# nicholasburden/pymarl

Hardware: NVIDIA B200
Metric: qmix_learner_episodes_per_sec (higher is better)
Workload: dtype bf16 (fp32 accumulate)

## Files before the change

pymarl_b200/csrc/api.cu:

```cuda
#include <cstdlib>
#include <stdarg.h>
#include <string.h>
#include <stdlib.h>
#include <atomic>
#include <mutex>
#include <vector>
#include <cuda_bf16.h>
#include "common.cuh"
#include "gru_tc.cuh"
#include "mixer_tc.cuh"

namespace pmb {

int gru_fwd_dispatch(const pmb_dims* d, const AgentParams& p, int64_t R, int nt, const float* x, const float* h0,
                     float* h_stash, float* gates, float* q, float* h_last, cudaStream_t s);
int gru_bwd_dispatch(const pmb_dims* d, const pmb_batch* b, const AgentParams& p, const float* x,
                     const float* h_stash, float* gates, const float* d_chosen, float* dpre1, cudaStream_t s,
                     const float* dq_full = nullptr);
int64_t scatter_scratch_bytes(const pmb_dims* d);
int scatter_grads_dispatch(const pmb_dims* d, const pmb_batch* b, const float* h_stash, const float* dpre1,
                           const float* d_chosen, AgentGrads gr, void* scratch, int64_t scratch_bytes, cudaStream_t s,
                           int ti_tiles = 0);
int launch_target_select(const pmb_dims* d, const pmb_batch* b, const float* q_on, const float* q_tg, float* chosen,
                         float* tmax, int32_t* cur_max, cudaStream_t s);
// ... 222 lines not shown
        T * R * A,
        T * R * A,
        M * N,
        M * N,
        qmix ? (tc_mix ? tc_raw_img_bytes(d) / 4 : M * C) : 0,
        (d->precision == PMB_PREC_BF16 && d->H == 64) ? T * n_tiles * ((d->O + 63) / 64) * ti : 0,
        iql ? 0 : M,
        iql ? 0 : M,
        M * W,
        iql ? 0 : M * N,
        tc_mix ? tc_state_img_bytes(d) / 4 : 0,
        (d->precision == PMB_PREC_BF16 && d->H == 64) ? (T + 1) * n_tiles * ti : 0,
        (d->precision == PMB_PREC_BF16 && d->H == 64) ? T * n_tiles * 256 : 0,
        0
    };
    WsPlan p;
    int64_t off = 0;
    for (int i = 0; i < 17; ++i) {
        p.off[i] = off;
        off += align_up(sizes[i] * 4, 256);
    }
    int64_t sc = agent_bwd_scratch(d);
    int64_t mb = mixer_bwd_scratch_bytes(d);
    if (mb > sc) sc = mb;
    if (d->precision == PMB_PREC_BF16) {
        int64_t f = tc_fc1_scratch_bytes(d);
        if (f > sc) sc = f;
        int64_t g = 131072 + tc_gru_bwd2_partial_bytes((int)ceil_div((int64_t)d->B * d->N, 128));
        if (g > sc) sc = g;
        int64_t a2 = tc_atb_ti_scratch_bytes(d->T, (int)ceil_div((int64_t)d->B * d->N, 128), d->O);
        if (a2 > sc) sc = a2;
        if (tc_agent_dw_scratch_bytes() > sc) sc = tc_agent_dw_scratch_bytes();
        if (tc_mix) {
            int64_t m2 = tc_mixer_scratch_bytes(d); if (m2 > sc) sc = m2;
            int64_t m3 = tc_mixer_bwd_img_scratch_bytes(d); if (m3 > sc) sc = m3;
        }
    }
    if (sc < 65536) sc = 65536;
    p.off[17] = off;
    p.scratch_bytes = align_up(sc, 256);
    p.mixdw_bytes = (tc_mix && d->H == 64) ? tc_mixer_dw_scratch_bytes(d) : 0;
    p.sched_bytes = skip_padding(d) ? skip_schedule_bytes(d->B, d->T, (int)n_tiles) : 0;
    p.total = off + p.scratch_bytes + p.mixdw_bytes + p.sched_bytes;
    return p;
}

void fill_views(const pmb_dims* d, void* ws, const WsPlan& p, pmb_ws_views* v) {
    char* base = static_cast<char*>(ws);
    auto f = [&](int i) { return reinterpret_cast<float*>(base + p.off[i]); };
    const bool iql = d->mixer == PMB_MIXER_NONE;
    v->x_on = f(0); v->x_tg = f(1); v->h_stash = f(2); v->gates = f(3); v->q_on = f(4); v->q_tg = f(5);
    v->chosen = f(6); v->tmax = f(7); v->raw_on = f(8); v->raw_tg = f(8);
    v->q_tot = iql ? v->chosen : f(10);
    v->t_tot = iql ? v->tmax : f(11);
    v->g = f(12);
    v->d_chosen = iql ? v->g : f(13);
    v->scratch = f(17);
    v->relu_mask = f(16);
    v->state_img = f(14);
    v->h_tg = f(15);
    v->scratch_bytes = p.scratch_bytes;
    v->obs_img = f(9);
    v->ep_order = nullptr;
    v->tile_steps = nullptr;
    if (p.sched_bytes) {
        SkipSchedule S = skip_schedule_views(base + p.total - p.sched_bytes, d->B, d->T, (int)ceil_div((int64_t)d->B * d->N, 128));
        v->ep_order = S.ep_order;
// ... 429 lines not shown
        }
        if ((rc = tc_gru_fwd2(img(0), img(24576), on.b_ih, on.b_hh, x_on_ti, h_ti, g_ti, R, d->T, n_tiles, s, tpc, tile_steps)))
            return rc;
        if (fork_tg) {
            PMB_CUDA(cudaStreamWaitEvent(s, side->join, 0));
        } else {
            PHASE(s, "gru_unroll_fwd_target_tc");
            if ((rc = tc_gru_fwd2(img(57344), img(57344 + 24576), tg.b_ih, tg.b_hh, x_tg_ti, hg_ti, nullptr, R, d->T, n_tiles,
                                  s, 2, tile_steps))) return rc;
        }
        PHASE(s, "q_select_tc");
        if ((rc = tc_q_select(d, b, img(49152), img(57344 + 49152), on.fc2_b, tg.fc2_b, h_ti, hg_ti, n_tiles, v.chosen,
                              v.tmax, (hp->keep_q & 1) ? v.q_on : nullptr, (hp->keep_q & 1) ? v.q_tg : nullptr, s, live_items,
                              n_live, tile_steps))) return rc;
    } else {
        PHASE(s, "fc1_fwd_online");
        if ((rc = fc1_fwd(d, b, 0, d->T, on, v.x_on, s))) return rc;
        PHASE(s, "fc1_fwd_target");
        if ((rc = fc1_fwd(d, b, 0, d->T, tg, v.x_tg, s))) return rc;
    }
    if (!tc_agent) {
        PHASE(s, "gru_unroll_fwd_online");
        if ((rc = gru_fwd_dispatch(d, on, R, d->T, v.x_on, nullptr, v.h_stash, v.gates, v.q_on, nullptr, s))) return rc;
        PHASE(s, "gru_unroll_fwd_target");
        if ((rc = gru_fwd_dispatch(d, tg, R, d->T, v.x_tg, nullptr, nullptr, nullptr, v.q_tg, nullptr, s))) return rc;
    }
    if (!tc_agent) {
        PHASE(s, "target_select");
        if ((rc = launch_target_select(d, b, v.q_on, v.q_tg, v.chosen, v.tmax, nullptr, s))) return rc;
    }
    uint8_t* state_img = reinterpret_cast<uint8_t*>(v.state_img);
    uint8_t* raw_img = reinterpret_cast<uint8_t*>(v.raw_on);
    if (tc_mixer) {
        PHASE(s, "state_to_images");
        if ((rc = tc_state_to_images(d, b, state_img, s))) return rc;
        PHASE(s, "mixer_fwd_target_tc");
        if ((rc = tc_mixer_fwd_img(d, mixer_params(d, flat_target + L.n_agent), state_img, v.tmax, 1, nullptr, v.t_tot,
                                   v.scratch, v.scratch_bytes, s))) return rc;
        PHASE(s, "mixer_fwd_online_tc");
        if ((rc = tc_mixer_fwd_img(d, mixer_params(d, flat_p + L.n_agent), state_img, v.chosen, 0, raw_img, v.q_tot,
                                   v.scratch, v.scratch_bytes, s))) return rc;
    } else if (d->mixer != PMB_MIXER_NONE) {
        PHASE(s, "mixer_fwd_target");
        if ((rc = launch_mixer_fwd(d, b, flat_target + L.n_agent, v.tmax, 1, v.raw_tg, v.t_tot, s))) return rc;
        PHASE(s, "mixer_fwd_online");
        if ((rc = launch_mixer_fwd(d, b, flat_p + L.n_agent, v.chosen, 0, v.raw_on, v.q_tot, s))) return rc;
    }
    PHASE(s, "td_loss");
    if ((rc = launch_td_loss(d, b, v.q_tot, v.t_tot, hp->gamma, v.g, stats, s, reinterpret_cast<double*>(v.scratch),
                             v.scratch_bytes))) return rc;
    if (hp->keep_q & 2) {
        PHASE(s, "end");
        return PMB_OK;
    }
    PHASE(s, "mixer_bwd");
    SideStream* side_dw = nullptr;
    if (tc_mixer) {
        static const int dw_fork_mode = []() { const char* e = getenv("PMB_DW_FORK"); return e ? atoi(e) : -1; }();
        const int free_sms = sm_count() - n_tiles;
        const bool fork_dw = tc_agent && plan.mixdw_bytes > 0 && dw_fork_mode != 0 && free_sms >= tc_mixer_dw_ctas(d);
        if (!fork_dw) {
            if ((rc = tc_mixer_bwd_img(d, mixer_params(d, flat_p + L.n_agent), state_img, raw_img, v.chosen, v.g, v.d_chosen,
                                       flat_g + L.offset[PMB_P_HW1_W], flat_g + L.offset[PMB_P_HW1_B],
                                       flat_g + L.offset[PMB_P_V2_W], flat_g + L.offset[PMB_P_V2_B], v.scratch,
                                       v.scratch_bytes, s))) return rc;
        } else {
            if ((rc = tc_mixer_bwd_img_dq(d, mixer_params(d, flat_p + L.n_agent), raw_img, v.chosen, v.g, v.d_chosen,
                                          flat_g + L.offset[PMB_P_V2_W], flat_g + L.offset[PMB_P_V2_B], v.scratch,
                                          v.scratch_bytes, s))) return rc;
            if ((rc = side_stream(&side_dw))) return rc;
            PMB_CUDA(cudaEventRecord(side_dw->fork2, s));
            PMB_CUDA(cudaStreamWaitEvent(side_dw->stream, side_dw->fork2, 0));
            if ((rc = tc_mixer_dw(d, state_img, raw_img, flat_g + L.offset[PMB_P_HW1_W], flat_g + L.offset[PMB_P_HW1_B],
                                  reinterpret_cast<char*>(v.scratch) + plan.scratch_bytes, plan.mixdw_bytes, free_sms,
// ... 253 lines not shown
```

pymarl_b200/csrc/mixer_tc.cuh:

```cuda
#pragma once
#include <cuda_bf16.h>
#include "common.cuh"

namespace pmb {

int64_t tc_packed_elems(int Ncols, int K);
int tc_pack_w(const float* const* ptrs, const int* rows, const int* lds, int nseg, int K, __nv_bfloat16* out,
              cudaStream_t s, int n_chunks_min = 0);

inline int tc_state_chunks(const pmb_dims* d) { return (d->S + 1 + 63) / 64; }
inline int tc_mix_cblks(const pmb_dims* d) { return (d->N + 3 + 1) / 2; }
inline int64_t tc_mix_row_tiles(const pmb_dims* d) { return ((int64_t)d->B * d->T + 127) / 128; }
inline int64_t tc_state_img_bytes(const pmb_dims* d) { return tc_mix_row_tiles(d) * tc_state_chunks(d) * 16384; }
inline int64_t tc_raw_img_bytes(const pmb_dims* d) { return tc_mix_row_tiles(d) * tc_mix_cblks(d) * 16384; }

int64_t tc_mixer_scratch_bytes(const pmb_dims* d);
int tc_state_to_images(const pmb_dims* d, const pmb_batch* b, uint8_t* img, cudaStream_t s);
int tc_mixer_fwd_img(const pmb_dims* d, const MixerParams& mp, const uint8_t* state_img, const float* agent_qs, int t_off,
                     uint8_t* raw_img, float* q_tot, void* scratch, int64_t scratch_bytes, cudaStream_t s);

int64_t tc_mixer_bwd_img_scratch_bytes(const pmb_dims* d);
int tc_mixer_bwd_img_dq(const pmb_dims* d, const MixerParams& mp, uint8_t* raw_img, const float* agent_qs, const float* g,
                        float* d_agent_qs, float* gv2_w, float* gv2_b, void* scratch, int64_t scratch_bytes, cudaStream_t s);
int tc_mixer_dw_ctas(const pmb_dims* d);
int64_t tc_mixer_dw_scratch_bytes(const pmb_dims* d);
int tc_mixer_dw(const pmb_dims* d, const uint8_t* state_img, const uint8_t* raw_img, float* gw_cat, float* gb_cat,
                void* scratch, int64_t scratch_bytes, int ctas_avail, cudaStream_t s);
int tc_mixer_bwd_img(const pmb_dims* d, const MixerParams& mp, const uint8_t* state_img, uint8_t* raw_img,
                     const float* agent_qs, const float* g, float* d_agent_qs, float* gw_cat, float* gb_cat, float* gv2_w,
                     float* gv2_b, void* scratch, int64_t scratch_bytes, cudaStream_t s);

}
```

pymarl_b200/csrc/tc_common.cuh:

```cuda
#pragma once
#include <cuda_bf16.h>
#include <stdint.h>

namespace pmb {
namespace tc {

__device__ __forceinline__ uint32_t smem_u32(const void* p) { return (uint32_t)__cvta_generic_to_shared(p); }

__device__ __forceinline__ void mbar_init(uint64_t* bar, uint32_t count) {
    asm volatile("mbarrier.init.shared::cta.b64 [%0], %1;" ::"r"(smem_u32(bar)), "r"(count) : "memory");
}
__device__ __forceinline__ void fence_barrier_init() {
    asm volatile("fence.mbarrier_init.release.cluster;" ::: "memory");
}
__device__ __forceinline__ void mbar_arrive(uint64_t* bar) {
    asm volatile("mbarrier.arrive.shared::cta.b64 _, [%0];" ::"r"(smem_u32(bar)) : "memory");
}
__device__ __forceinline__ void mbar_arrive_expect_tx(uint64_t* bar, uint32_t bytes) {
    asm volatile("mbarrier.arrive.expect_tx.shared::cta.b64 _, [%0], %1;" ::"r"(smem_u32(bar)), "r"(bytes) : "memory");
}
__device__ __forceinline__ bool mbar_try_wait(uint64_t* bar, uint32_t parity) {
    uint32_t ok;
    asm volatile(
        "{\n\t.reg .pred p;\n\t"
// ... 4 lines not shown
        : "memory");
    return ok != 0;
}
__device__ __forceinline__ void mbar_wait(uint64_t* bar, uint32_t parity) {
    while (!mbar_try_wait(bar, parity)) {
    }
}

typedef unsigned long long f32x2;
__device__ __forceinline__ f32x2 f2_make(float lo, float hi) {
    f32x2 r;
    asm("mov.b64 %0, {%1, %2};" : "=l"(r) : "f"(lo), "f"(hi));
    return r;
}
__device__ __forceinline__ void f2_split(f32x2 v, float& lo, float& hi) { asm("mov.b64 {%0, %1}, %2;" : "=f"(lo), "=f"(hi) : "l"(v)); }
__device__ __forceinline__ f32x2 f2_from_bf16x2(uint32_t w) { return f2_make(__uint_as_float(w << 16), __uint_as_float(w & 0xffff0000u)); }
__device__ __forceinline__ f32x2 f2_fma(f32x2 a, f32x2 b, f32x2 c) {
    f32x2 d;
    asm("fma.rn.f32x2 %0, %1, %2, %3;" : "=l"(d) : "l"(a), "l"(b), "l"(c));
    return d;
}
__device__ __forceinline__ f32x2 f2_mul(f32x2 a, f32x2 b) {
    f32x2 d;
    asm("mul.rn.f32x2 %0, %1, %2;" : "=l"(d) : "l"(a), "l"(b));
    return d;
}
__device__ __forceinline__ f32x2 f2_add(f32x2 a, f32x2 b) {
    f32x2 d;
    asm("add.rn.f32x2 %0, %1, %2;" : "=l"(d) : "l"(a), "l"(b));
    return d;
}

__device__ __forceinline__ void fence_proxy_async_smem() { asm volatile("fence.proxy.async.shared::cta;" ::: "memory"); }

__device__ __forceinline__ void bulk_copy_g2s(void* dst_smem, const void* src_gmem, uint32_t bytes, uint64_t* bar) {
    asm volatile("cp.async.bulk.shared::cluster.global.mbarrier::complete_tx::bytes [%0], [%1], %2, [%3];" ::"r"(
                     smem_u32(dst_smem)),
                 "l"(src_gmem), "r"(bytes), "r"(smem_u32(bar))
                 : "memory");
}

__device__ __forceinline__ void bulk_copy_s2g(void* dst_gmem, const void* src_smem, uint32_t bytes) {
    asm volatile("cp.async.bulk.global.shared::cta.bulk_group [%0], [%1], %2;" ::"l"(dst_gmem), "r"(smem_u32(src_smem)),
                 "r"(bytes)
                 : "memory");
}
__device__ __forceinline__ void bulk_commit_group() { asm volatile("cp.async.bulk.commit_group;" ::: "memory"); }
template <int N>
__device__ __forceinline__ void bulk_wait_group_read() { asm volatile("cp.async.bulk.wait_group.read %0;" ::"n"(N) : "memory"); }
template <int N>
__device__ __forceinline__ void bulk_wait_group() { asm volatile("cp.async.bulk.wait_group %0;" ::"n"(N) : "memory"); }

__device__ __forceinline__ void tmem_alloc(uint32_t* slot_smem, uint32_t ncols) {
    asm volatile("tcgen05.alloc.cta_group::1.sync.aligned.shared::cta.b32 [%0], %1;" ::"r"(smem_u32(slot_smem)), "r"(ncols)
                 : "memory");
    asm volatile("tcgen05.relinquish_alloc_permit.cta_group::1.sync.aligned;" ::: "memory");
}
__device__ __forceinline__ void tmem_dealloc(uint32_t taddr, uint32_t ncols) {
    asm volatile("tcgen05.dealloc.cta_group::1.sync.aligned.b32 %0, %1;" ::"r"(taddr), "r"(ncols) : "memory");
}
__device__ __forceinline__ void pdl_launch_dependents() { asm volatile("griddepcontrol.launch_dependents;" ::: "memory"); }
__device__ __forceinline__ void pdl_wait() { asm volatile("griddepcontrol.wait;" ::: "memory"); }

__device__ __forceinline__ void tc_fence_before() { asm volatile("tcgen05.fence::before_thread_sync;" ::: "memory"); }
__device__ __forceinline__ void tc_fence_after() { asm volatile("tcgen05.fence::after_thread_sync;" ::: "memory"); }
__device__ __forceinline__ void tmem_wait_ld() { asm volatile("tcgen05.wait::ld.sync.aligned;" ::: "memory"); }
// ... 75 lines not shown
```

pymarl_b200/csrc/tc_gemm.cu:

```cuda
#include <cstdlib>
#include <algorithm>
#include "common.cuh"
#include "tc_common.cuh"
#include "mixer_tc.cuh"

namespace pmb {
namespace tc {

constexpr int BM = 128;
constexpr int BK = 64;
constexpr int BN_MAX = 256;
constexpr int STAGES = 4;
constexpr int A_STAGE_BYTES = BM * 128;
constexpr int W_STAGE_BYTES = BN_MAX * 128;
constexpr int N_EPI_WARPS = 4, MMA_WARP = 4, WLOAD_WARP = 5, FIRST_PROD_WARP = 6, N_PROD_WARPS = 8;
constexpr int THREADS = 32 * (FIRST_PROD_WARP + N_PROD_WARPS);
constexpr int SMEM_BYTES = 1024  + STAGES * (A_STAGE_BYTES + W_STAGE_BYTES) + 256;

struct GemmParams {
    const float* A;
    RowMap amap;
    int64_t M;
    int K;
    int n_chunks;
    const __nv_bfloat16* Wp;
    int Ncols;
    int64_t tm_R, tm_Rpad;
    int tm_N, tm_T;
    uint8_t* a_img_out;
    const uint8_t* a_img;
};

__host__ __device__ inline int pass_cols(int Ncols, int p) {
    int left = Ncols - p * BN_MAX;
    return left < BN_MAX ? left : BN_MAX;
}
__host__ __device__ inline int64_t packed_tile_offset(int Ncols, int n_chunks, int p, int c) {
    return ((int64_t)p * BN_MAX * n_chunks + (int64_t)c * pass_cols(Ncols, p)) * BK;
}

struct PackSegs {
    const float* ptr[4];
    int rows[4];
    int ld[4];
    int nseg;
};

__global__ void __launch_bounds__(256)
pack_w_kernel(PackSegs segs, int K, int n_chunks, int Ncols, __nv_bfloat16* __restrict__ out) {
    const int64_t total = (int64_t)Ncols * n_chunks * 8;
    int64_t i = (int64_t)blockIdx.x * blockDim.x + threadIdx.x;
    if (i >= total) return;
    int j = (int)(i & 7);
    int64_t rc = i >> 3;
    int col = (int)(rc % Ncols);
    int c = (int)(rc / Ncols);
    int p = col / BN_MAX, r = col - p * BN_MAX;
    const float* src = nullptr;
    int rr = col;
    for (int s = 0; s < segs.nseg; ++s) {
        if (rr < segs.rows[s]) { src = segs.ptr[s] ? segs.ptr[s] + (int64_t)rr * segs.ld[s] : nullptr; break; }
        rr -= segs.rows[s];
    }
    uint32_t w[4];
#pragma unroll
    for (int q = 0; q < 4; ++q) {
        int k = c * BK + j * 8 + q * 2;
        float lo = (src && k < K) ? src[k] : 0.f;
        float hi = (src && k + 1 < K) ? src[k + 1] : 0.f;
        w[q] = pack_bf16x2(lo, hi);
    }
    char* tile = reinterpret_cast<char*>(out + packed_tile_offset(Ncols, n_chunks, p, c));
    *reinterpret_cast<uint4*>(tile + sw128_offset((uint32_t)r, (uint32_t)j)) = make_uint4(w[0], w[1], w[2], w[3]);
}

template <class Epi>
__global__ void __launch_bounds__(THREADS, 1) tc_gemm_kernel(GemmParams P, Epi epi) {
    extern __shared__ uint8_t smem_raw[];
    uint8_t* smem = reinterpret_cast<uint8_t*>((reinterpret_cast<uintptr_t>(smem_raw) + 1023) & ~(uintptr_t)1023);
    uint8_t* a_stage = smem;
    uint8_t* w_stage = smem + STAGES * A_STAGE_BYTES;
    uint64_t* bars = reinterpret_cast<uint64_t*>(smem + STAGES * (A_STAGE_BYTES + W_STAGE_BYTES));
    uint64_t* full = bars;
    uint64_t* empty = bars + STAGES;
    uint64_t* tfull = bars + 2 * STAGES;
    uint64_t* tempty = tfull + 2;
    uint32_t* tmem_slot = reinterpret_cast<uint32_t*>(tempty + 2);

    const int warp = threadIdx.x >> 5, lane = threadIdx.x & 31;
    if (threadIdx.x == 0) {
        for (int s = 0; s < STAGES; ++s) { mbar_init(&full[s], P.a_img ? 1 : N_PROD_WARPS + 1); mbar_init(&empty[s], 1); }
        for (int b = 0; b < 2; ++b) { mbar_init(&tfull[b], 1); mbar_init(&tempty[b], N_EPI_WARPS); }
        fence_barrier_init();
    }
    if (warp == MMA_WARP) tmem_alloc(tmem_slot, 512);
    tc_fence_before();
    __syncthreads();
    tc_fence_after();
    const uint32_t tmem_base = *tmem_slot;

    const int64_t n_tiles = (P.M + BM - 1) / BM;
    const int n_pass = (P.Ncols + BN_MAX - 1) / BN_MAX;

    if (warp >= FIRST_PROD_WARP) {
        const int pw = warp - FIRST_PROD_WARP;
        uint32_t it = 0;
        if (P.a_img == nullptr)
        for (int64_t tile = blockIdx.x; tile < n_tiles; tile += gridDim.x) {
            const float* myptr = nullptr;
            if (lane < BM / N_PROD_WARPS) {
                int64_t row = tile * BM + pw + N_PROD_WARPS * lane;
                if (row < P.M) {
                    if (P.tm_R > 0) {
                        const int64_t t = row / P.tm_Rpad, pp = row - t * P.tm_Rpad;
                        if (pp < P.tm_R) {
                            const int64_t bb = pp / P.tm_N, nn = pp - bb * P.tm_N;
                            myptr = P.A + P.amap.offset((bb * P.tm_T + t) * P.tm_N + nn);
                        }
                    } else {
                        myptr = P.A + P.amap.offset(row);
                    }
                }
            }
            for (int p = 0; p < n_pass; ++p) {
                for (int c = 0; c < P.n_chunks; ++c, ++it) {
                    const int s = it % STAGES;
                    mbar_wait(&empty[s], ((it / STAGES) & 1) ^ 1);
                    uint8_t* dst = a_stage + s * A_STAGE_BYTES;
                    const int k = c * BK + 2 * lane;
                    float v0[BM / N_PROD_WARPS], v1[BM / N_PROD_WARPS];
#pragma unroll
                    for (int l = 0; l < BM / N_PROD_WARPS; ++l) {
                        const float* rp = reinterpret_cast<const float*>(
                            __shfl_sync(0xffffffffu, reinterpret_cast<uintptr_t>(myptr), l));
                        float a = 0.f, b = 0.f;
                        if (rp != nullptr) {
                            if (k + 1 < P.K && ((reinterpret_cast<uintptr_t>(rp + k) & 7) == 0)) {
                                float2 t = __ldg(reinterpret_cast<const float2*>(rp + k));
                                a = t.x; b = t.y;
                            } else {
                                if (k < P.K) a = __ldg(rp + k);
                                if (k + 1 < P.K) b = __ldg(rp + k + 1);
                            }
                        }
                        v0[l] = a; v1[l] = b;
                    }
                    uint8_t* gimg = (P.a_img_out && p == 0)
                                        ? P.a_img_out + ((int64_t)tile * P.n_chunks + c) * A_STAGE_BYTES : nullptr;
#pragma unroll
                    for (int l = 0; l < BM / N_PROD_WARPS; ++l) {
                        const uint32_t r = pw + N_PROD_WARPS * l;
                        const uint32_t off = sw128_offset(r, lane >> 2) + (lane & 3) * 4;
                        const uint32_t w = pack_bf16x2(v0[l], v1[l]);
                        *reinterpret_cast<uint32_t*>(dst + off) = w;
                        if (gimg) *reinterpret_cast<uint32_t*>(gimg + off) = w;
                    }
                    fence_proxy_async_smem();
                    __syncwarp();
                    if (lane == 0) mbar_arrive(&full[s]);
                }
            }
        }
    } else if (warp == WLOAD_WARP) {
        if (lane == 0) {
            uint32_t it = 0;
            for (int64_t tile = blockIdx.x; tile < n_tiles; tile += gridDim.x)
                for (int p = 0; p < n_pass; ++p) {
                    const uint32_t bytes = (uint32_t)pass_cols(P.Ncols, p) * 128u;
                    for (int c = 0; c < P.n_chunks; ++c, ++it) {
                        const int s = it % STAGES;
                        mbar_wait(&empty[s], ((it / STAGES) & 1) ^ 1);
                        mbar_arrive_expect_tx(&full[s], bytes + (P.a_img ? A_STAGE_BYTES : 0));
                        bulk_copy_g2s(w_stage + s * W_STAGE_BYTES, P.Wp + packed_tile_offset(P.Ncols, P.n_chunks, p, c),
                                      bytes, &full[s]);
                        if (P.a_img)
                            bulk_copy_g2s(a_stage + s * A_STAGE_BYTES, P.a_img + ((int64_t)tile * P.n_chunks + c) * A_STAGE_BYTES,
                                          A_STAGE_BYTES, &full[s]);
                    }
                }
        }
    } else if (warp == MMA_WARP) {
        if (lane == 0) {
            uint32_t it = 0, acc_it = 0;
            for (int64_t tile = blockIdx.x; tile < n_tiles; tile += gridDim.x)
                for (int p = 0; p < n_pass; ++p, ++acc_it) {
                    const int b = acc_it & 1;
                    const uint32_t idesc = umma_idesc_bf16(BM, pass_cols(P.Ncols, p), 0, 0);
                    mbar_wait(&tempty[b], ((acc_it >> 1) & 1) ^ 1);
                    tc_fence_after();
                    const uint32_t tmem_d = tmem_base + (uint32_t)b * BN_MAX;
                    for (int c = 0; c < P.n_chunks; ++c, ++it) {
                        const int s = it % STAGES;
                        mbar_wait(&full[s], (it / STAGES) & 1);
                        tc_fence_after();
                        const uint32_t a_addr = smem_u32(a_stage + s * A_STAGE_BYTES);
                        const uint32_t w_addr = smem_u32(w_stage + s * W_STAGE_BYTES);
#pragma unroll
                        for (int kk = 0; kk < BK / 16; ++kk) {
                            umma_bf16(tmem_d, umma_desc_sw128(a_addr + kk * 32, 16, 1024),
                                      umma_desc_sw128(w_addr + kk * 32, 16, 1024), idesc, (c | kk) != 0);
                        }
                        umma_commit(&empty[s]);
                    }
                    umma_commit(&tfull[b]);
                }
        }
    } else {
        uint32_t acc_it = 0;
        for (int64_t tile = blockIdx.x; tile < n_tiles; tile += gridDim.x) {
            const int64_t m = tile * BM + warp * 32 + lane;
            const bool valid = m < P.M;
            typename Epi::Row row;
            epi.begin(row, m, valid);
            epi.attach(row, smem + STAGES * (A_STAGE_BYTES + W_STAGE_BYTES) + 256 + warp * (Epi::EXTRA_SMEM / N_EPI_WARPS));
            for (int p = 0; p < n_pass; ++p, ++acc_it) {
                const int b = acc_it & 1;
                const int ncols = pass_cols(P.Ncols, p);
                mbar_wait(&tfull[b], (acc_it >> 1) & 1);
                tc_fence_after();
                const uint32_t taddr = tmem_base + (uint32_t)b * BN_MAX + ((uint32_t)(warp * 32) << 16);
                for (int g = 0; g < ncols; g += 32) {
                    uint32_t v[32];
                    tmem_ld_32x32(taddr + g, v);
                    tmem_wait_ld();
                    epi.cols(row, m, valid, p * BN_MAX + g, v);
                }
                tc_fence_before();
                __syncwarp();
                if (lane == 0) mbar_arrive(&tempty[b]);
            }
            epi.end(row, m, valid);
        }
        epi.finish();
    }
    tc_fence_before();
    __syncthreads();
    if (warp == MMA_WARP) {
        tc_fence_after();
        tmem_dealloc(tmem_base, 512);
    }
}

struct PlainEpi {
    static constexpr int EXTRA_SMEM = 0;
    template <class R> __device__ void attach(R&, uint8_t*) const {}
    __device__ void finish() const {}
    struct Row {};
    float* C; int64_t ldc; const float* bias; int Nreal;
    __device__ void begin(Row&, int64_t, bool) const {}
    __device__ void cols(Row&, int64_t m, bool valid, int col0, const uint32_t (&v)[32]) const {
        if (!valid) return;
#pragma unroll
        for (int j = 0; j < 32; ++j)
            if (col0 + j < Nreal) C[m * ldc + col0 + j] = __uint_as_float(v[j]) + (bias ? bias[col0 + j] : 0.f);
    }
    __device__ void end(Row&, int64_t, bool) const {}
};

struct Fc1Epi {
    static constexpr int EXTRA_SMEM = 0;
    template <class R> __device__ void attach(R&, uint8_t*) const {}
    __device__ void finish() const {}
    struct Row { int64_t out_off; int n; int a_prev; };
    const float* tab_act;
    const float* tab_id;
    const int64_t* actions; int64_t actions_sb;
// ... 141 lines not shown
            if (col0 & 32) flush(r, col0 >> 6);
        }
        if (grp < N) {
            const float qn = r.mq >= 0 ? __ldg(agent_qs + r.mq * N + grp) : 0.f;
#pragma unroll
            for (int e = 0; e < 32; ++e) r.hidden[e] = fmaf(qn, fabsf(raw[e]), r.hidden[e]);
        } else if (grp == N) {
#pragma unroll
            for (int e = 0; e < 32; ++e) {
                float pre = r.hidden[e] + raw[e];
                r.hidden[e] = pre > 0.f ? pre : expm1f(pre);
            }
        } else if (grp == N + 1) {
#pragma unroll
            for (int e = 0; e < 32; ++e) r.y = fmaf(r.hidden[e], fabsf(raw[e]), r.y);
        } else if (grp == N + 2) {
#pragma unroll
            for (int e = 0; e < 32; ++e) r.y = fmaf(fmaxf(raw[e], 0.f), __ldg(v2_w + e), r.y);
        }
    }
    __device__ void end(Row& r, int64_t, bool) const {
        if (r.mq >= 0) q_tot[r.mq] = r.y + __ldg(v2_b);
        if (r.img) {
            if ((N + 3) & 1) flush(r, (N + 3) >> 1);
            if ((threadIdx.x & 31) == 0) bulk_wait_group_read<0>();
            __syncwarp();
        }
    }
    __device__ void finish() const {
        if ((threadIdx.x & 31) == 0) bulk_wait_group<0>();
    }
};

template <class Epi>
int launch_tc_gemm(const GemmParams& P, const Epi& epi, cudaStream_t s) {
    if (P.M <= 0) return PMB_OK;
    auto kern = tc_gemm_kernel<Epi>;
    PMB_SMEM_ATTR(kern, SMEM_BYTES + Epi::EXTRA_SMEM);
    int64_t n_tiles = (P.M + BM - 1) / BM;
    int grid = (int)(n_tiles < sm_count() ? n_tiles : sm_count());
    kern<<<grid, THREADS, SMEM_BYTES + Epi::EXTRA_SMEM, s>>>(P, epi);
    PMB_LAUNCH_CHECK("tc_gemm_kernel");
    return PMB_OK;
}


namespace fs {
constexpr int MAX_CHUNKS = 5;
constexpr int group_rows_of(int es) { return 64 / es; }
template <int ES> constexpr int group_rows() { return group_rows_of(ES); }
constexpr int RUN_SLACK = 272;
constexpr int N_SLOTS = 3;
constexpr int N_SLOTS_1NET = 5;
#ifndef PMB_FC1_NCONV
#define PMB_FC1_NCONV 8
#endif
constexpr int N_EPI = 4, MMA_W = 4, PROD_W = 5, N_CONV = PMB_FC1_NCONV;
constexpr int threads_for(int ns) { return 32 * (PROD_W + ns + N_CONV); }
static_assert(group_rows<4>() % N_CONV == 0 && group_rows<2>() % N_CONV == 0, "group rows must divide over the converter warps");
static_assert(BM % group_rows<4>() == 0 && BM % group_rows<2>() == 0, "group rows must divide the tile");
static_assert(group_rows<4>() <= 32 && group_rows<2>() <= 32, "the producer writes one row table entry per lane");
}

struct Fc1StreamParams {
    const int64_t* ep_index;
    const uint8_t* obs; int64_t obs_sb;
    const __nv_bfloat16* Wp;
    uint8_t* obs_img;
    int64_t R;
    int T, N, O, n_tiles, n_chunks, slot_bytes;
    int fold_id;
    const uint4* tab_act16;
    const float* tab_id;
    const int64_t* actions; int64_t actions_sb;
    const int64_t* filled;  int64_t filled_sb;
    uint8_t* x_on; uint8_t* x_tg;
    uint32_t* relu_mask;
// ... 859 lines not shown
                PMB_FC1_STREAM_LAUNCH(5)
            }
#undef PMB_FC1_STREAM_LAUNCH
            set_error("tc_fc1: %d k-chunks", n_chunks);
            return PMB_ERR_INVALID;
        }
        if (b->ep_index || live_items) { set_error("tc_fc1: ep_index and live items need the streaming kernel (obs dim <= 320)"); return PMB_ERR_INVALID; }
        return tc::launch_tc_gemm(P, epi, s);
    }
    if (b->ep_index || live_items) { set_error("tc_fc1: ep_index and live items are not supported without tile images"); return PMB_ERR_INVALID; }
    tc::Fc1Epi epi{tab_act, tab_id, b->actions, b->actions_sb, b->filled, b->filled_sb, x_on, x_tg,
                   t0, nt, d->N, d->A, d->obs_last_action, (int64_t)d->B * d->N};
    return tc::launch_tc_gemm(P, epi, s);
}
int64_t tc_fc1_scratch_bytes(const pmb_dims* d) {
    return align_up(tc_packed_elems(128, d->O) * 2, 256) + align_up((int64_t)2 * d->A * 64 * 4, 256) +
           align_up((int64_t)2 * d->N * 64 * 4, 256) + align_up((int64_t)d->A * 128 * 2, 256);
}

__global__ void mix_bias_perm_kernel(const float* __restrict__ b_cat, int N, float* __restrict__ out) {
    int i = blockIdx.x * blockDim.x + threadIdx.x;
    int C = (N + 3) * 32;
    if (i >= C) return;
    int grp = i >> 5, e = i & 31;
    int src_grp = grp < N ? grp : (grp == N ? N + 1 : (grp == N + 1 ? N : N + 2));
    out[i] = b_cat[src_grp * 32 + e];
}

int64_t tc_mixer_scratch_bytes(const pmb_dims* d) {
    const int C = (d->N + 3) * 32;
    return align_up(tc_packed_elems((int)align_up(C, 32), d->S + 1) * 2, 256) + align_up((int64_t)C * 4, 256);
}

__global__ void __launch_bounds__(256)
state_to_images_kernel(const float* __restrict__ state, int64_t state_sb, const int64_t* __restrict__ ep_index, int64_t BT,
                       int T, int S, int n_chunks, uint8_t* __restrict__ img) {
    const int64_t total = ((BT + 127) / 128) * 128 * (int64_t)n_chunks * 8;
    int64_t i = (int64_t)blockIdx.x * blockDim.x + threadIdx.x;
    if (i >= total) return;
    const int j = (int)(i & 7);
    int64_t q = i >> 3;
    const int r = (int)(q & 127);
    q >>= 7;
    const int c = (int)(q % n_chunks);
    const int64_t tile = q / n_chunks;
    const int64_t m = tile * 128 + r;
    float f[8] = {0.f, 0.f, 0.f, 0.f, 0.f, 0.f, 0.f, 0.f};
    if (m < BT) {
        const int64_t b = m / T;
        const int t = (int)(m - b * T);
        const float* src = state + ep_row(ep_index, b) * state_sb + (int64_t)t * S + c * 64 + j * 8;
        const int nv = S - (c * 64 + j * 8);
        if (nv >= 8 && (reinterpret_cast<uintptr_t>(src) & 7) == 0) {
#pragma unroll
            for (int e = 0; e < 4; ++e) {
                const float2 v = __ldg(reinterpret_cast<const float2*>(src) + e);
                f[2 * e] = v.x; f[2 * e + 1] = v.y;
            }
        } else {
#pragma unroll
            for (int e = 0; e < 8; ++e) {
                if (e < nv) f[e] = __ldg(src + e);
                else if (e == nv) f[e] = 1.0f;
            }
        }
    }
    *reinterpret_cast<uint4*>(img + (tile * n_chunks + c) * 16384 + tc::sw128_offset((uint32_t)r, (uint32_t)j)) =
        make_uint4(tc::pack_bf16x2(f[0], f[1]), tc::pack_bf16x2(f[2], f[3]), tc::pack_bf16x2(f[4], f[5]),
                   tc::pack_bf16x2(f[6], f[7]));
}

int tc_state_to_images(const pmb_dims* d, const pmb_batch* b, uint8_t* img, cudaStream_t s) {
    const int64_t BT = (int64_t)d->B * d->T;
    const int n_chunks = tc_state_chunks(d);
    const int64_t total = ((BT + 127) / 128) * 128 * (int64_t)n_chunks * 8;
    state_to_images_kernel<<<(unsigned)ceil_div(total, 256), 256, 0, s>>>(b->state, b->state_sb, b->ep_index, BT, d->T, d->S, n_chunks,
                                                                                  img);
    PMB_LAUNCH_CHECK("state_to_images_kernel");
    return PMB_OK;
}

int tc_mixer_fwd_img(const pmb_dims* d, const MixerParams& mp, const uint8_t* state_img, const float* agent_qs, int t_off,
                     uint8_t* raw_img, float* q_tot, void* scratch, int64_t scratch_bytes, cudaStream_t s) {
    const int N = d->N, S = d->S, C = (N + 3) * 32;
    const int n_chunks = tc_state_chunks(d);
    if (scratch_bytes < tc_mixer_scratch_bytes(d)) { set_error("tc_mixer: scratch too small"); return PMB_ERR_WORKSPACE; }
    __nv_bfloat16* wp = static_cast<__nv_bfloat16*>(scratch);
    float* bias = reinterpret_cast<float*>(static_cast<char*>(scratch) + align_up(tc_packed_elems(C, S + 1) * 2, 256));
    const float* ptrs[4] = {mp.w_cat, mp.w_cat + (int64_t)(N + 1) * 32 * S, mp.w_cat + (int64_t)N * 32 * S,
                            mp.w_cat + (int64_t)(N + 2) * 32 * S};
    int rows[4] = {N * 32, 32, 32, 32}, lds[4] = {S, S, S, S};
    int rc = tc_pack_w(ptrs, rows, lds, 4, S, wp, s, n_chunks);
    if (rc) return rc;
    mix_bias_perm_kernel<<<(unsigned)ceil_div(C, 256), 256, 0, s>>>(mp.b_cat, N, bias);
    PMB_LAUNCH_CHECK("mix_bias_perm_kernel");
    const int64_t BT = (int64_t)d->B * d->T;
    tc::GemmParams P{nullptr, dense_map(0), ((BT + 127) / 128) * 128, n_chunks * 64, n_chunks, wp, C,
                     0, 0, 0, 0, nullptr, state_img};
    tc::MixImgEpi epi{bias, agent_qs, mp.v2_w, mp.v2_b, q_tot, raw_img, N, d->T, t_off, tc_mix_cblks(d), BT};
    return tc::launch_tc_gemm(P, epi, s);
}

}
```

Baseline: 149,300.

## Fuse state image build and target/online mixer forward GEMMs into one kernel

Replaces the separate state_to_images kernel and two mixer forward GEMM launches with a single paired tensor-core kernel. Producer warps convert state rows to swizzled bf16 images in global memory and signal the weight loader through new mbarriers. Each A tile is then consumed by both the target and online weight sets, with two epilogues running back to back. This cuts launches and one A-image pass, but needs twice the mixer scratch and serialises image writing with TMA reads through a global proxy fence.

```diff
diff --git a/pymarl_b200/csrc/api.cu b/pymarl_b200/csrc/api.cu
--- a/pymarl_b200/csrc/api.cu
+++ b/pymarl_b200/csrc/api.cu
@@ -278,7 +278,7 @@
         if (a2 > sc) sc = a2;
         if (tc_agent_dw_scratch_bytes() > sc) sc = tc_agent_dw_scratch_bytes();
         if (tc_mix) {
-            int64_t m2 = tc_mixer_scratch_bytes(d); if (m2 > sc) sc = m2;
+            int64_t m2 = 2 * tc_mixer_scratch_bytes(d); if (m2 > sc) sc = m2;
             int64_t m3 = tc_mixer_bwd_img_scratch_bytes(d); if (m3 > sc) sc = m3;
         }
     }
@@ -774,14 +774,22 @@
     uint8_t* state_img = reinterpret_cast<uint8_t*>(v.state_img);
     uint8_t* raw_img = reinterpret_cast<uint8_t*>(v.raw_on);
     if (tc_mixer) {
-        PHASE(s, "state_to_images");
-        if ((rc = tc_state_to_images(d, b, state_img, s))) return rc;
-        PHASE(s, "mixer_fwd_target_tc");
-        if ((rc = tc_mixer_fwd_img(d, mixer_params(d, flat_target + L.n_agent), state_img, v.tmax, 1, nullptr, v.t_tot,
-                                   v.scratch, v.scratch_bytes, s))) return rc;
-        PHASE(s, "mixer_fwd_online_tc");
-        if ((rc = tc_mixer_fwd_img(d, mixer_params(d, flat_p + L.n_agent), state_img, v.chosen, 0, raw_img, v.q_tot,
-                                   v.scratch, v.scratch_bytes, s))) return rc;
+        const char* e_fuse = getenv("PMB_MIX_FUSE");
+        if (!(e_fuse && e_fuse[0] == '0')) {
+            PHASE(s, "mixer_fwd_both_tc");
+            if ((rc = tc_mixer_fwd_both(d, b, mixer_params(d, flat_target + L.n_agent), mixer_params(d, flat_p + L.n_agent),
+                                        state_img, v.tmax, v.chosen, raw_img, v.t_tot, v.q_tot, v.scratch, v.scratch_bytes,
+                                        s))) return rc;
+        } else {
+            PHASE(s, "state_to_images");
+            if ((rc = tc_state_to_images(d, b, state_img, s))) return rc;
+            PHASE(s, "mixer_fwd_target_tc");
+            if ((rc = tc_mixer_fwd_img(d, mixer_params(d, flat_target + L.n_agent), state_img, v.tmax, 1, nullptr, v.t_tot,
+                                       v.scratch, v.scratch_bytes, s))) return rc;
+            PHASE(s, "mixer_fwd_online_tc");
+            if ((rc = tc_mixer_fwd_img(d, mixer_params(d, flat_p + L.n_agent), state_img, v.chosen, 0, raw_img, v.q_tot,
+                                       v.scratch, v.scratch_bytes, s))) return rc;
+        }
     } else if (d->mixer != PMB_MIXER_NONE) {
         PHASE(s, "mixer_fwd_target");
         if ((rc = launch_mixer_fwd(d, b, flat_target + L.n_agent, v.tmax, 1, v.raw_tg, v.t_tot, s))) return rc;
diff --git a/pymarl_b200/csrc/mixer_tc.cuh b/pymarl_b200/csrc/mixer_tc.cuh
--- a/pymarl_b200/csrc/mixer_tc.cuh
+++ b/pymarl_b200/csrc/mixer_tc.cuh
@@ -18,6 +18,9 @@
 int tc_state_to_images(const pmb_dims* d, const pmb_batch* b, uint8_t* img, cudaStream_t s);
 int tc_mixer_fwd_img(const pmb_dims* d, const MixerParams& mp, const uint8_t* state_img, const float* agent_qs, int t_off,
                      uint8_t* raw_img, float* q_tot, void* scratch, int64_t scratch_bytes, cudaStream_t s);
+int tc_mixer_fwd_both(const pmb_dims* d, const pmb_batch* b, const MixerParams& tg, const MixerParams& on, uint8_t* state_img,
+                      const float* tmax, const float* chosen, uint8_t* raw_img, float* t_tot, float* q_tot, void* scratch,
+                      int64_t scratch_bytes, cudaStream_t s);
 
 int64_t tc_mixer_bwd_img_scratch_bytes(const pmb_dims* d);
 int tc_mixer_bwd_img_dq(const pmb_dims* d, const MixerParams& mp, uint8_t* raw_img, const float* agent_qs, const float* g,
diff --git a/pymarl_b200/csrc/tc_common.cuh b/pymarl_b200/csrc/tc_common.cuh
--- a/pymarl_b200/csrc/tc_common.cuh
+++ b/pymarl_b200/csrc/tc_common.cuh
@@ -60,6 +60,7 @@
 }
 
 __device__ __forceinline__ void fence_proxy_async_smem() { asm volatile("fence.proxy.async.shared::cta;" ::: "memory"); }
+__device__ __forceinline__ void fence_proxy_async_global() { asm volatile("fence.proxy.async.global;" ::: "memory"); }
 
 __device__ __forceinline__ void bulk_copy_g2s(void* dst_smem, const void* src_gmem, uint32_t bytes, uint64_t* bar) {
     asm volatile("cp.async.bulk.shared::cluster.global.mbarrier::complete_tx::bytes [%0], [%1], %2, [%3];" ::"r"(
diff --git a/pymarl_b200/csrc/tc_gemm.cu b/pymarl_b200/csrc/tc_gemm.cu
--- a/pymarl_b200/csrc/tc_gemm.cu
+++ b/pymarl_b200/csrc/tc_gemm.cu
@@ -16,6 +16,38 @@
 constexpr int N_EPI_WARPS = 4, MMA_WARP = 4, WLOAD_WARP = 5, FIRST_PROD_WARP = 6, N_PROD_WARPS = 8;
 constexpr int THREADS = 32 * (FIRST_PROD_WARP + N_PROD_WARPS);
 constexpr int SMEM_BYTES = 1024  + STAGES * (A_STAGE_BYTES + W_STAGE_BYTES) + 256;
+
+struct StateSrc {
+    const float* state; int64_t state_sb;
+    const int64_t* ep_index;
+    int64_t BT;
+    int T, S;
+};
+__device__ __forceinline__ void state_load(const StateSrc& st, int64_t m, int c, int j, float (&f)[8]) {
+#pragma unroll
+    for (int e = 0; e < 8; ++e) f[e] = 0.f;
+    if (m >= st.BT) return;
+    const int64_t b = m / st.T;
+    const int t = (int)(m - b * st.T);
+    const float* src = st.state + ep_row(st.ep_index, b) * st.state_sb + (int64_t)t * st.S + c * 64 + j * 8;
+    const int nv = st.S - (c * 64 + j * 8);
+    if (nv >= 8 && (reinterpret_cast<uintptr_t>(src) & 7) == 0) {
+#pragma unroll
+        for (int e = 0; e < 4; ++e) {
+            const float2 v = __ldg(reinterpret_cast<const float2*>(src) + e);
+            f[2 * e] = v.x; f[2 * e + 1] = v.y;
+        }
+    } else {
+#pragma unroll
+        for (int e = 0; e < 8; ++e) {
+            if (e < nv) f[e] = __ldg(src + e);
+            else if (e == nv) f[e] = 1.0f;
+        }
+    }
+}
+__device__ __forceinline__ uint4 pack_bf16x8(const float (&f)[8]) {
+    return make_uint4(pack_bf16x2(f[0], f[1]), pack_bf16x2(f[2], f[3]), pack_bf16x2(f[4], f[5]), pack_bf16x2(f[6], f[7]));
+}
 
 struct GemmParams {
     const float* A;
@@ -29,6 +61,8 @@
     int tm_N, tm_T;
     uint8_t* a_img_out;
     const uint8_t* a_img;
+    const __nv_bfloat16* Wp2;
+    StateSrc st;
 };
 
 __host__ __device__ inline int pass_cols(int Ncols, int p) {
@@ -74,8 +108,8 @@
     *reinterpret_cast<uint4*>(tile + sw128_offset((uint32_t)r, (uint32_t)j)) = make_uint4(w[0], w[1], w[2], w[3]);
 }
 
-template <class Epi>
-__global__ void __launch_bounds__(THREADS, 1) tc_gemm_kernel(GemmParams P, Epi epi) {
+template <class Epi, bool PAIR>
+__global__ void __launch_bounds__(THREADS, 1) tc_gemm_kernel(GemmParams P, Epi epi, Epi epi2) {
     extern __shared__ uint8_t smem_raw[];
     uint8_t* smem = reinterpret_cast<uint8_t*>((reinterpret_cast<uintptr_t>(smem_raw) + 1023) & ~(uintptr_t)1023);
     uint8_t* a_stage = smem;
@@ -85,12 +119,16 @@
     uint64_t* empty = bars + STAGES;
     uint64_t* tfull = bars + 2 * STAGES;
     uint64_t* tempty = tfull + 2;
-    uint32_t* tmem_slot = reinterpret_cast<uint32_t*>(tempty + 2);
+    uint64_t* ready = tempty + 2;
+    uint64_t* taken = ready + 1;
+    uint32_t* tmem_slot = reinterpret_cast<uint32_t*>(taken + 1);
 
     const int warp = threadIdx.x >> 5, lane = threadIdx.x & 31;
     if (threadIdx.x == 0) {
         for (int s = 0; s < STAGES; ++s) { mbar_init(&full[s], P.a_img ? 1 : N_PROD_WARPS + 1); mbar_init(&empty[s], 1); }
         for (int b = 0; b < 2; ++b) { mbar_init(&tfull[b], 1); mbar_init(&tempty[b], N_EPI_WARPS); }
+        mbar_init(ready, 32 * N_PROD_WARPS);
+        mbar_init(taken, 1);
         fence_barrier_init();
     }
     if (warp == MMA_WARP) tmem_alloc(tmem_slot, 512);
@@ -101,11 +139,31 @@
 
     const int64_t n_tiles = (P.M + BM - 1) / BM;
     const int n_pass = (P.Ncols + BN_MAX - 1) / BN_MAX;
+    constexpr int n_w = PAIR ? 2 : 1;
 
     if (warp >= FIRST_PROD_WARP) {
         const int pw = warp - FIRST_PROD_WARP;
         uint32_t it = 0;
-        if (P.a_img == nullptr)
+        if constexpr (PAIR) {
+            constexpr int NT = 32 * N_PROD_WARPS, U = BM * 8 / NT;
+            const int tid = threadIdx.x - 32 * FIRST_PROD_WARP;
+            uint32_t jl = 0;
+            for (int64_t tile = blockIdx.x; tile < n_tiles; tile += gridDim.x, ++jl) {
+                if (jl > 0) mbar_wait(taken, (jl - 1) & 1);
+                uint8_t* img = const_cast<uint8_t*>(P.a_img) + tile * P.n_chunks * A_STAGE_BYTES;
+                for (int c = 0; c < P.n_chunks; ++c) {
+                    float f[U][8];
+#pragma unroll
+                    for (int u = 0; u < U; ++u) state_load(P.st, tile * BM + ((tid + u * NT) >> 3), c, tid & 7, f[u]);
+#pragma unroll
+                    for (int u = 0; u < U; ++u)
+                        *reinterpret_cast<uint4*>(img + c * A_STAGE_BYTES + sw128_offset((tid + u * NT) >> 3, tid & 7)) =
+                            pack_bf16x8(f[u]);
+                }
+                fence_proxy_async_global();
+                mbar_arrive(ready);
+            }
+        } else if (P.a_img == nullptr)
         for (int64_t tile = blockIdx.x; tile < n_tiles; tile += gridDim.x) {
             const float* myptr = nullptr;
             if (lane < BM / N_PROD_WARPS) {
@@ -163,27 +221,36 @@
         }
     } else if (warp == WLOAD_WARP) {
         if (lane == 0) {
-            uint32_t it = 0;
-            for (int64_t tile = blockIdx.x; tile < n_tiles; tile += gridDim.x)
-                for (int p = 0; p < n_pass; ++p) {
-                    const uint32_t bytes = (uint32_t)pass_cols(P.Ncols, p) * 128u;
-                    for (int c = 0; c < P.n_chunks; ++c, ++it) {
-                        const int s = it % STAGES;
-                        mbar_wait(&empty[s], ((it / STAGES) & 1) ^ 1);
-                        mbar_arrive_expect_tx(&full[s], bytes + (P.a_img ? A_STAGE_BYTES : 0));
-                        bulk_copy_g2s(w_stage + s * W_STAGE_BYTES, P.Wp + packed_tile_offset(P.Ncols, P.n_chunks, p, c),
-                                      bytes, &full[s]);
-                        if (P.a_img)
-                            bulk_copy_g2s(a_stage + s * A_STAGE_BYTES, P.a_img + ((int64_t)tile * P.n_chunks + c) * A_STAGE_BYTES,
-                                          A_STAGE_BYTES, &full[s]);
+            uint32_t it = 0, jl = 0;
+            for (int64_t tile = blockIdx.x; tile < n_tiles; tile += gridDim.x, ++jl) {
+                if (PAIR) {
+                    mbar_wait(ready, jl & 1);
+                    mbar_arrive(taken);
+                }
+                for (int w = 0; w < n_w; ++w)
+                    for (int p = 0; p < n_pass; ++p) {
+                        const uint32_t bytes = (uint32_t)pass_cols(P.Ncols, p) * 128u;
+                        const __nv_bfloat16* wsrc = w ? P.Wp2 : P.Wp;
+                        for (int c = 0; c < P.n_chunks; ++c, ++it) {
+                            const int s = it % STAGES;
+                            mbar_wait(&empty[s], ((it / STAGES) & 1) ^ 1);
+                            mbar_arrive_expect_tx(&full[s], bytes + (P.a_img ? A_STAGE_BYTES : 0));
+                            bulk_copy_g2s(w_stage + s * W_STAGE_BYTES, wsrc + packed_tile_offset(P.Ncols, P.n_chunks, p, c),
+                                          bytes, &full[s]);
+                            if (P.a_img)
+                                bulk_copy_g2s(a_stage + s * A_STAGE_BYTES,
+                                              P.a_img + ((int64_t)tile * P.n_chunks + c) * A_STAGE_BYTES, A_STAGE_BYTES,
+                                              &full[s]);
+                        }
                     }
-                }
+            }
         }
     } else if (warp == MMA_WARP) {
         if (lane == 0) {
             uint32_t it = 0, acc_it = 0;
             for (int64_t tile = blockIdx.x; tile < n_tiles; tile += gridDim.x)
-                for (int p = 0; p < n_pass; ++p, ++acc_it) {
+                for (int wp = 0; wp < n_w * n_pass; ++wp, ++acc_it) {
+                    const int p = wp % n_pass;
                     const int b = acc_it & 1;
                     const uint32_t idesc = umma_idesc_bf16(BM, pass_cols(P.Ncols, p), 0, 0);
                     mbar_wait(&tempty[b], ((acc_it >> 1) & 1) ^ 1);
@@ -207,12 +274,10 @@
         }
     } else {
         uint32_t acc_it = 0;
-        for (int64_t tile = blockIdx.x; tile < n_tiles; tile += gridDim.x) {
-            const int64_t m = tile * BM + warp * 32 + lane;
-            const bool valid = m < P.M;
+        auto run = [&](const Epi& e, int64_t m, bool valid) {
             typename Epi::Row row;
-            epi.begin(row, m, valid);
-            epi.attach(row, smem + STAGES * (A_STAGE_BYTES + W_STAGE_BYTES) + 256 + warp * (Epi::EXTRA_SMEM / N_EPI_WARPS));
+            e.begin(row, m, valid);
+            e.attach(row, smem + STAGES * (A_STAGE_BYTES + W_STAGE_BYTES) + 256 + warp * (Epi::EXTRA_SMEM / N_EPI_WARPS));
             for (int p = 0; p < n_pass; ++p, ++acc_it) {
                 const int b = acc_it & 1;
                 const int ncols = pass_cols(P.Ncols, p);
@@ -223,15 +288,22 @@
                     uint32_t v[32];
                     tmem_ld_32x32(taddr + g, v);
                     tmem_wait_ld();
-                    epi.cols(row, m, valid, p * BN_MAX + g, v);
+                    e.cols(row, m, valid, p * BN_MAX + g, v);
                 }
                 tc_fence_before();
                 __syncwarp();
                 if (lane == 0) mbar_arrive(&tempty[b]);
             }
-            epi.end(row, m, valid);
+            e.end(row, m, valid);
+        };
+        for (int64_t tile = blockIdx.x; tile < n_tiles; tile += gridDim.x) {
+            const int64_t m = tile * BM + warp * 32 + lane;
+            const bool valid = m < P.M;
+            run(epi, m, valid);
+            if (PAIR) run(epi2, m, valid);
         }
         epi.finish();
+        if (PAIR) epi2.finish();
     }
     tc_fence_before();
     __syncthreads();
@@ -439,17 +511,19 @@
     }
 };
 
-template <class Epi>
-int launch_tc_gemm(const GemmParams& P, const Epi& epi, cudaStream_t s) {
+template <class Epi, bool PAIR>
+int launch_tc_gemm(const GemmParams& P, const Epi& epi, cudaStream_t s, const Epi& epi2) {
     if (P.M <= 0) return PMB_OK;
-    auto kern = tc_gemm_kernel<Epi>;
+    auto kern = tc_gemm_kernel<Epi, PAIR>;
     PMB_SMEM_ATTR(kern, SMEM_BYTES + Epi::EXTRA_SMEM);
     int64_t n_tiles = (P.M + BM - 1) / BM;
     int grid = (int)(n_tiles < sm_count() ? n_tiles : sm_count());
-    kern<<<grid, THREADS, SMEM_BYTES + Epi::EXTRA_SMEM, s>>>(P, epi);
+    kern<<<grid, THREADS, SMEM_BYTES + Epi::EXTRA_SMEM, s>>>(P, epi, epi2);
     PMB_LAUNCH_CHECK("tc_gemm_kernel");
     return PMB_OK;
 }
+template <class Epi>
+int launch_tc_gemm(const GemmParams& P, const Epi& epi, cudaStream_t s) { return launch_tc_gemm<Epi, false>(P, epi, s, epi); }
 
 
 namespace fs {
@@ -1375,10 +1449,8 @@
     return align_up(tc_packed_elems((int)align_up(C, 32), d->S + 1) * 2, 256) + align_up((int64_t)C * 4, 256);
 }
 
-__global__ void __launch_bounds__(256)
-state_to_images_kernel(const float* __restrict__ state, int64_t state_sb, const int64_t* __restrict__ ep_index, int64_t BT,
-                       int T, int S, int n_chunks, uint8_t* __restrict__ img) {
-    const int64_t total = ((BT + 127) / 128) * 128 * (int64_t)n_chunks * 8;
+__global__ void __launch_bounds__(256) state_to_images_kernel(tc::StateSrc st, int n_chunks, uint8_t* __restrict__ img) {
+    const int64_t total = ((st.BT + 127) / 128) * 128 * (int64_t)n_chunks * 8;
     int64_t i = (int64_t)blockIdx.x * blockDim.x + threadIdx.x;
     if (i >= total) return;
     const int j = (int)(i & 7);
@@ -1387,61 +1459,70 @@
     q >>= 7;
     const int c = (int)(q % n_chunks);
     const int64_t tile = q / n_chunks;
-    const int64_t m = tile * 128 + r;
-    float f[8] = {0.f, 0.f, 0.f, 0.f, 0.f, 0.f, 0.f, 0.f};
-    if (m < BT) {
-        const int64_t b = m / T;
-        const int t = (int)(m - b * T);
-        const float* src = state + ep_row(ep_index, b) * state_sb + (int64_t)t * S + c * 64 + j * 8;
-        const int nv = S - (c * 64 + j * 8);
-        if (nv >= 8 && (reinterpret_cast<uintptr_t>(src) & 7) == 0) {
-#pragma unroll
-            for (int e = 0; e < 4; ++e) {
-                const float2 v = __ldg(reinterpret_cast<const float2*>(src) + e);
-                f[2 * e] = v.x; f[2 * e + 1] = v.y;
-            }
-        } else {
-#pragma unroll
-            for (int e = 0; e < 8; ++e) {
-                if (e < nv) f[e] = __ldg(src + e);
-                else if (e == nv) f[e] = 1.0f;
-            }
-        }
-    }
-    *reinterpret_cast<uint4*>(img + (tile * n_chunks + c) * 16384 + tc::sw128_offset((uint32_t)r, (uint32_t)j)) =
-        make_uint4(tc::pack_bf16x2(f[0], f[1]), tc::pack_bf16x2(f[2], f[3]), tc::pack_bf16x2(f[4], f[5]),
-                   tc::pack_bf16x2(f[6], f[7]));
+    float f[8];
+    tc::state_load(st, tile * 128 + r, c, j, f);
+    *reinterpret_cast<uint4*>(img + (tile * n_chunks + c) * 16384 + tc::sw128_offset((uint32_t)r, (uint32_t)j)) = tc::pack_bf16x8(f);
+}
+
+static tc::StateSrc state_src(const pmb_dims* d, const pmb_batch* b) {
+    return tc::StateSrc{b->state, b->state_sb, b->ep_index, (int64_t)d->B * d->T, d->T, d->S};
 }
 
 int tc_state_to_images(const pmb_dims* d, const pmb_batch* b, uint8_t* img, cudaStream_t s) {
-    const int64_t BT = (int64_t)d->B * d->T;
     const int n_chunks = tc_state_chunks(d);
-    const int64_t total = ((BT + 127) / 128) * 128 * (int64_t)n_chunks * 8;
-    state_to_images_kernel<<<(unsigned)ceil_div(total, 256), 256, 0, s>>>(b->state, b->state_sb, b->ep_index, BT, d->T, d->S, n_chunks,
-                                                                                  img);
+    const int64_t total = tc_mix_row_tiles(d) * 128 * (int64_t)n_chunks * 8;
+    state_to_images_kernel<<<(unsigned)ceil_div(total, 256), 256, 0, s>>>(state_src(d, b), n_chunks, img);
     PMB_LAUNCH_CHECK("state_to_images_kernel");
     return PMB_OK;
 }
 
-int tc_mixer_fwd_img(const pmb_dims* d, const MixerParams& mp, const uint8_t* state_img, const float* agent_qs, int t_off,
-                     uint8_t* raw_img, float* q_tot, void* scratch, int64_t scratch_bytes, cudaStream_t s) {
+static int pack_mixer(const pmb_dims* d, const MixerParams& mp, void* scratch, __nv_bfloat16** wp, float** bias, cudaStream_t s) {
     const int N = d->N, S = d->S, C = (N + 3) * 32;
-    const int n_chunks = tc_state_chunks(d);
-    if (scratch_bytes < tc_mixer_scratch_bytes(d)) { set_error("tc_mixer: scratch too small"); return PMB_ERR_WORKSPACE; }
-    __nv_bfloat16* wp = static_cast<__nv_bfloat16*>(scratch);
-    float* bias = reinterpret_cast<float*>(static_cast<char*>(scratch) + align_up(tc_packed_elems(C, S + 1) * 2, 256));
+    *wp = static_cast<__nv_bfloat16*>(scratch);
+    *bias = reinterpret_cast<float*>(static_cast<char*>(scratch) + align_up(tc_packed_elems(C, S + 1) * 2, 256));
     const float* ptrs[4] = {mp.w_cat, mp.w_cat + (int64_t)(N + 1) * 32 * S, mp.w_cat + (int64_t)N * 32 * S,
                             mp.w_cat + (int64_t)(N + 2) * 32 * S};
     int rows[4] = {N * 32, 32, 32, 32}, lds[4] = {S, S, S, S};
-    int rc = tc_pack_w(ptrs, rows, lds, 4, S, wp, s, n_chunks);
+    int rc = tc_pack_w(ptrs, rows, lds, 4, S, *wp, s, tc_state_chunks(d));
     if (rc) return rc;
-    mix_bias_perm_kernel<<<(unsigned)ceil_div(C, 256), 256, 0, s>>>(mp.b_cat, N, bias);
+    mix_bias_perm_kernel<<<(unsigned)ceil_div(C, 256), 256, 0, s>>>(mp.b_cat, N, *bias);
     PMB_LAUNCH_CHECK("mix_bias_perm_kernel");
-    const int64_t BT = (int64_t)d->B * d->T;
-    tc::GemmParams P{nullptr, dense_map(0), ((BT + 127) / 128) * 128, n_chunks * 64, n_chunks, wp, C,
-                     0, 0, 0, 0, nullptr, state_img};
-    tc::MixImgEpi epi{bias, agent_qs, mp.v2_w, mp.v2_b, q_tot, raw_img, N, d->T, t_off, tc_mix_cblks(d), BT};
-    return tc::launch_tc_gemm(P, epi, s);
-}
-
-}
+    return PMB_OK;
+}
+
+static tc::GemmParams mixer_gemm_params(const pmb_dims* d, const __nv_bfloat16* wp, const uint8_t* state_img) {
+    const int n_chunks = tc_state_chunks(d);
+    return tc::GemmParams{nullptr, dense_map(0), tc_mix_row_tiles(d) * 128, n_chunks * 64, n_chunks, wp, (d->N + 3) * 32,
+                          0, 0, 0, 0, nullptr, state_img};
+}
+
+int tc_mixer_fwd_img(const pmb_dims* d, const MixerParams& mp, const uint8_t* state_img, const float* agent_qs, int t_off,
+                     uint8_t* raw_img, float* q_tot, void* scratch, int64_t scratch_bytes, cudaStream_t s) {
+    if (scratch_bytes < tc_mixer_scratch_bytes(d)) { set_error("tc_mixer: scratch too small"); return PMB_ERR_WORKSPACE; }
+    __nv_bfloat16* wp; float* bias;
+    int rc = pack_mixer(d, mp, scratch, &wp, &bias, s);
+    if (rc) return rc;
+    tc::MixImgEpi epi{bias, agent_qs, mp.v2_w, mp.v2_b, q_tot, raw_img, d->N, d->T, t_off, tc_mix_cblks(d), (int64_t)d->B * d->T};
+    return tc::launch_tc_gemm(mixer_gemm_params(d, wp, state_img), epi, s);
+}
+
+int tc_mixer_fwd_both(const pmb_dims* d, const pmb_batch* b, const MixerParams& tg, const MixerParams& on, uint8_t* state_img,
+                      const float* tmax, const float* chosen, uint8_t* raw_img, float* t_tot, float* q_tot, void* scratch,
+                      int64_t scratch_bytes, cudaStream_t s) {
+    const int64_t half = tc_mixer_scratch_bytes(d);
+    if (scratch_bytes < 2 * half) { set_error("tc_mixer: scratch too small"); return PMB_ERR_WORKSPACE; }
+    __nv_bfloat16 *wp_tg, *wp_on; float *bias_tg, *bias_on;
+    int rc = pack_mixer(d, tg, scratch, &wp_tg, &bias_tg, s);
+    if (rc) return rc;
+    if ((rc = pack_mixer(d, on, static_cast<char*>(scratch) + half, &wp_on, &bias_on, s))) return rc;
+    tc::GemmParams P = mixer_gemm_params(d, wp_tg, state_img);
+    P.Wp2 = wp_on;
+    P.st = state_src(d, b);
+    const int N = d->N, T = d->T, n_cblk = tc_mix_cblks(d);
+    const int64_t BT = (int64_t)d->B * T;
+    tc::MixImgEpi epi_tg{bias_tg, tmax, tg.v2_w, tg.v2_b, t_tot, nullptr, N, T, 1, n_cblk, BT};
+    tc::MixImgEpi epi_on{bias_on, chosen, on.v2_w, on.v2_b, q_tot, raw_img, N, T, 0, n_cblk, BT};
+    return tc::launch_tc_gemm<tc::MixImgEpi, true>(P, epi_tg, s, epi_on);
+}
+
+}
```

After: 150,300 (median of 6 runs). About the same (+0.7%).
